# ru-wang/slam-plus-plus

Measured on AMD Instinct MI355X. Metric: Λ-solve block-nnz/sec + batch GN iters/sec, Venice BA, 1→8 MI355X, higher is better.
Workload: dtype f64; 1 GPU; venice871-shaped synthetic BA (871 cams, 530304 points, 2838740 observations, LM-damped); nnzb=3369915, n=1596138, mode=schur+dense, n_reduced=5226, schur_pairs=12875640, parallelism=single GPU

## Files before the change

### include/spp_hip.h

```cpp
#ifndef SPP_HIP_H
#define SPP_HIP_H

#include <stddef.h>
#include <stdint.h>

#ifdef __cplusplus
extern "C" {
#endif

#define SPP_OK            0
#define SPP_NOT_POSDEF    1
#define SPP_E_BADARG     -1
#define SPP_E_NOMEM      -2
#define SPP_E_HIP        -3
#define SPP_E_NO_DEVICE  -4
#define SPP_E_STATE      -5
#define SPP_E_UNSUPPORTED -6

#define SPP_MODE_AUTO     0
#define SPP_MODE_SPARSE   1
#define SPP_MODE_SCHUR    2
#define SPP_MODE_SCHUR_SPARSE 3

#define SPP_FLAG_PROFILE  1
// ... 3 lines not shown

spp_ctx *spp_create(int device, int flags);
void spp_destroy(spp_ctx *ctx);
int spp_free_memory(spp_ctx *ctx);
int spp_last_error(const spp_ctx *ctx, char *buf, size_t buf_size);
double *spp_host_staging(spp_ctx *ctx, int64_t n_doubles);
int spp_set_stream(spp_ctx *ctx, void *hip_stream);
int spp_synchronize(spp_ctx *ctx);

int spp_analyze(spp_ctx *ctx, int64_t nb, const int64_t *h_col_ptr, const int64_t *h_row_idx,
	const int64_t *h_blk_off, const int32_t *h_dim, int mode);

int spp_set_shard(spp_ctx *ctx, int rank, int world_size);

#define SPP_MODE_SCHUR_MIS 4

#define SPP_INFO_MODE           0
#define SPP_INFO_N              1
#define SPP_INFO_NNZB           2
#define SPP_INFO_NVALS          3
#define SPP_INFO_FACTOR_NNZ     4
#define SPP_INFO_FACTOR_FLOPS   5
#define SPP_INFO_N_REDUCED      6
#define SPP_INFO_N_POSES        7
#define SPP_INFO_N_LANDMARKS    8
#define SPP_INFO_SCHUR_PAIRS    9
#define SPP_INFO_N_OBS          10
#define SPP_INFO_SOLVE_BYTES    11
#define SPP_INFO_N_SUPERNODES   12
#define SPP_INFO_N_LEVELS       13
#define SPP_INFO_S_LD           14
#define SPP_INFO_S_NNZB         15
#define SPP_INFO_DENSE_STREAMED 16
int spp_get_info(const spp_ctx *ctx, int what, int64_t *out);
int spp_get_ordering(const spp_ctx *ctx, int64_t *h_order);

#define SPP_ORDER_AMD 0
#define SPP_ORDER_ND  1
int spp_block_ordering(int64_t nb, const int64_t *col_ptr, const int64_t *row_idx, int method, int64_t *h_order);

int spp_schur_plan_host(int64_t nb, const int32_t *dim, const int64_t *col_ptr, const int64_t *row_idx, int shard_rank,
	int shard_world, int sparse_S, int64_t *out, double *seconds);

int spp_factor_solve(spp_ctx *ctx, const double *h_vals, double *h_rhs_inout);

int spp_factor_solve_device(spp_ctx *ctx, const double *d_vals, double *d_rhs_inout);

int spp_schur_buffer_size(const spp_ctx *ctx, int64_t *n_doubles);
int spp_schur_form(spp_ctx *ctx, const double *d_vals, const double *d_rhs, double *d_S_rhs);
int spp_schur_finish(spp_ctx *ctx, const double *d_vals, double *d_S_rhs, double *d_rhs_inout);
int spp_schur_packed_size(const spp_ctx *ctx, int64_t *n_doubles);
int spp_schur_pack(spp_ctx *ctx, const double *d_S_rhs, double *d_packed);
int spp_schur_unpack(spp_ctx *ctx, const double *d_packed, double *d_S_rhs);

int spp_assemble_analyze(spp_ctx *ctx, int64_t nv, const int32_t *h_dim,
	int64_t ne, const int64_t *h_v0, const int64_t *h_v1, int d0, int d1, int rd,
	int64_t unary_vertex);
int spp_assemble_get_structure(const spp_ctx *ctx, int64_t *h_col_ptr, int64_t *h_row_idx,
	int64_t *h_blk_off);
int spp_assemble_device(spp_ctx *ctx, const double *d_J0, const double *d_J1,
	const double *d_Omega, const double *d_r, double damping, double *d_vals_out, double *d_eta_out);
int spp_assemble_set_edge_weights(spp_ctx *ctx, const double *d_w);
int spp_edge_robust_weights_device(spp_ctx *ctx, int64_t n_edges, int rd, int kind, double scale, double param,
	const double *d_r, double *d_w_out);

int spp_se2_linearize_device(spp_ctx *ctx, int64_t n_edges, const int32_t *d_v0, const int32_t *d_v1,
// ... 72 lines not shown
```

### slam_plus_plus_amd/api.py

```python
import ctypes
import os

import numpy as np

_HERE = os.path.dirname(os.path.abspath(__file__))
LIB_PATH = os.environ.get("SPP_LIB") or os.path.join(_HERE, "libspp_hip.so")

SPP_OK, SPP_NOT_POSDEF = 0, 1
MODE_AUTO, MODE_SPARSE, MODE_SCHUR, MODE_SCHUR_SPARSE, MODE_SCHUR_MIS = 0, 1, 2, 3, 4
FLAG_PROFILE = 1
INFO = dict(MODE=0, N=1, NNZB=2, NVALS=3, FACTOR_NNZ=4, FACTOR_FLOPS=5, N_REDUCED=6, N_POSES=7,
            N_LANDMARKS=8, SCHUR_PAIRS=9, N_OBS=10, SOLVE_BYTES=11, N_SUPERNODES=12, N_LEVELS=13, S_LD=14, S_NNZB=15, DENSE_STREAMED=16)
PHASES = ["permute", "schur_inv", "schur_gemm", "schur_rhs", "factor", "trisolve", "backsubst", "assemble", "total"]

EXPORTS = [
    "spp_create", "spp_destroy", "spp_free_memory", "spp_last_error", "spp_host_staging", "spp_set_stream", "spp_synchronize",
    "spp_analyze", "spp_set_shard", "spp_get_info", "spp_get_ordering", "spp_factor_solve",
    "spp_factor_solve_device", "spp_schur_buffer_size", "spp_schur_form", "spp_schur_finish",
    "spp_schur_packed_size", "spp_schur_pack", "spp_schur_unpack",
    "spp_assemble_analyze", "spp_assemble_get_structure", "spp_assemble_device", "spp_assemble_set_edge_weights", "spp_device_malloc",
    "spp_device_free", "spp_memcpy_h2d", "spp_memcpy_d2h", "spp_memcpy_d2d", "spp_get_phase_ms", "spp_get_dominant_kernel",
    "spp_microbench_copy", "spp_microbench_mfma_f64", "spp_microbench_ctile", "spp_microbench_update", "spp_block_ordering", "spp_schur_plan_host", "spp_set_profiling", "spp_se2_linearize_device", "spp_se2_update_device", "spp_ba_linearize_device", "spp_ba_update_device", "spp_se3_linearize_device", "spp_se3_update_device", "spp_edge_chi2_device", "spp_edge_robust_weights_device", "spp_edge_hessian_maxdiag_device",
    "spp_lm_gain_denominator_device", "spp_dense_potrf_upper", "spp_dense_posv",
    "spp_dense_posv_masked", "spp_tile_mask_host", "spp_schur_tile_mask_host", "spp_tail_order_host", "spp_schur_cam_order_host",
    "spp_dense_gemm_tn_sub", "spp_dense_gemm_tn_sub_upper", "spp_dense_front_factor", "spp_version",
]

_lib = None
_c_i64p = ctypes.POINTER(ctypes.c_int64)
_c_i32p = ctypes.POINTER(ctypes.c_int32)
_c_f64p = ctypes.POINTER(ctypes.c_double)


class SppError(RuntimeError):
    """std::runtime_error of the C++ adapter (reference LinearSolver_Schur_GPU.cpp:734-797)."""


def load_library():
    global _lib
    if _lib is not None:
        return _lib
    if not os.path.exists(LIB_PATH):
        raise SppError("libspp_hip.so is not built: run `python -m slam_plus_plus_amd.build` "
                       "(hipcc --offload-arch=gfx950); there is no CPU fallback")
    lib = ctypes.CDLL(LIB_PATH)
# ... 444 lines not shown
```

### slam_plus_plus_amd/csrc/spp_api.cpp

```cpp

#include "spp_internal.h"
#include <string.h>
#include <new>

using namespace spp;

namespace spp {

void phases_reset(spp_ctx *ctx)
{
	if(!(ctx->flags & SPP_FLAG_PROFILE))
		return;
	if(!ctx->timer.created) {
		for(int i = 0; i < 2 * SPP_N_PHASES; ++ i)
			SPP_HIP_CHECK(hipEventCreate(&ctx->timer.ev[i]));
		ctx->timer.created = true;
	}
	for(int i = 0; i < SPP_N_PHASES; ++ i) {
		ctx->timer.used[i] = false;
		ctx->phase_ms[i] = 0;
	}
	ctx->dom_used = 0;
	ctx->dom_flops = 0;
}
// ... 326 lines not shown
	} else
		sparse_analyze(ctx, ctx->st);
	ctx->mode = chosen;
	clk.lap("plan + ordering");
	return SPP_OK;
	SPP_CATCH(ctx)
}

int spp_get_info(const spp_ctx *ctx, int what, int64_t *out)
{
	if(!ctx || !out)
		return SPP_E_BADARG;
	if(ctx->mode < 0 && what != SPP_INFO_NNZB && what != SPP_INFO_NVALS && what != SPP_INFO_N && what != SPP_INFO_DENSE_STREAMED)
		return SPP_E_STATE;
	switch(what) {
	case SPP_INFO_MODE: *out = (ctx->mode != SPP_MODE_SCHUR) ? ctx->mode : ctx->schur.mis ? SPP_MODE_SCHUR_MIS :
		ctx->schur.sparse_S ? SPP_MODE_SCHUR_SPARSE : SPP_MODE_SCHUR; break;
	case SPP_INFO_N: *out = ctx->st.n; break;
	case SPP_INFO_NNZB: *out = ctx->st.nnzb; break;
	case SPP_INFO_NVALS: *out = ctx->st.nvals; break;
	case SPP_INFO_FACTOR_NNZ: *out = ctx->factor_nnz; break;
	case SPP_INFO_FACTOR_FLOPS: *out = ctx->factor_flops; break;
	case SPP_INFO_N_REDUCED: *out = (ctx->mode == SPP_MODE_SCHUR) ? ctx->schur.n_red : 0; break;
	case SPP_INFO_N_POSES: *out = (ctx->mode == SPP_MODE_SCHUR) ? ctx->schur.nc : ctx->st.nb; break;
	case SPP_INFO_N_LANDMARKS: *out = (ctx->mode == SPP_MODE_SCHUR) ? ctx->schur.nl : 0; break;
	case SPP_INFO_SCHUR_PAIRS: *out = (ctx->mode == SPP_MODE_SCHUR) ? ctx->schur.n_pairs : 0; break;
	case SPP_INFO_N_OBS: *out = (ctx->mode == SPP_MODE_SCHUR) ? ctx->schur.no : 0; break;
	case SPP_INFO_SOLVE_BYTES: *out = ctx->solve_bytes; break;
	case SPP_INFO_N_SUPERNODES: *out = ctx->sparse ? sparse_info(ctx, what) : 0; break;
	case SPP_INFO_N_LEVELS: *out = ctx->sparse ? sparse_info(ctx, what) : 0; break;
	case SPP_INFO_S_LD: *out = (ctx->mode == SPP_MODE_SCHUR && !ctx->schur.sparse_S) ? ctx->schur.ld : 0; break;
	case SPP_INFO_S_NNZB: *out = (ctx->mode == SPP_MODE_SCHUR) ? ctx->schur.n_sblk : 0; break;
	case SPP_INFO_DENSE_STREAMED: *out = ctx->dense.tail_rows_last; break;
	default: return SPP_E_BADARG;
	}
	return SPP_OK;
}

int spp_get_ordering(const spp_ctx *ctx, int64_t *h_order)
{
	if(!ctx || !h_order)
		return SPP_E_BADARG;
	if(ctx->mode < 0)
		return SPP_E_STATE;
	for(size_t i = 0; i < ctx->order.size(); ++ i)
		h_order[i] = ctx->order[i];
	return SPP_OK;
}

int spp_block_ordering(int64_t nb, const int64_t *col_ptr, const int64_t *row_idx, int method, int64_t *h_order)
{
	if(nb <= 0 || !col_ptr || !row_idx || !h_order || (method != SPP_ORDER_AMD && method != SPP_ORDER_ND))
		return SPP_E_BADARG;
	try {
		for(int64_t j = 0; j < nb; ++ j)
			for(int64_t p = col_ptr[j]; p < col_ptr[j + 1]; ++ p)
				if(row_idx[p] < 0 || row_idx[p] > j)
					return SPP_E_BADARG;
		std::vector<int64_t> order;
		if(method == SPP_ORDER_AMD)
			min_degree_order(nb, col_ptr, row_idx, order);
		else
			nested_dissection_order(nb, col_ptr, row_idx, order);
		for(int64_t k = 0; k < nb; ++ k)
			h_order[k] = order[k];
		return SPP_OK;
// ... 692 lines not shown
```

### slam_plus_plus_amd/csrc/spp_internal.h

```cpp
#pragma once

#include <hip/hip_runtime.h>
#include <stdint.h>
#include <string>
#include <vector>
#include <sys/mman.h>
#include <utility>
#include <new>
#include <exception>
#include <thread>
#include <stdexcept>
#include <algorithm>
#include <string.h>
#include <chrono>
#include <stdio.h>
#include <stdlib.h>
#include "../../include/spp_hip.h"
#include "spp_switches.h"

namespace spp {

struct Error : std::runtime_error {
	int code;
	Error(int c, const std::string &what) : std::runtime_error(what), code(c) {}
// ... 152 lines not shown
	int32_t kind;
	int32_t a_tr;
	int64_t dst;
	int64_t aoff;
};

struct SchurDims {
	int dp = 0, dl = 0;
	int64_t nc = 0, nl = 0;
	int64_t nl_total = 0;
	int64_t no = 0;
	int64_t n_red = 0, ld = 0;
	int64_t n_sblk = 0;
	int64_t n_pairs = 0;
	int64_t n_items = 0, n_multi = 0;
	int32_t xcd_max_items = 0;
	bool u_landmark_major = true;
	bool factored = true;
};

struct SchurPlan : SchurDims {
	bool add_A = true;
	bool sparse_S = false;
	bool mis = false;
	Structure s_st;
	DevBuf<int64_t> sblk_voff;
	std::vector<int64_t> pose_block;
	std::vector<int64_t> lm_block;
	std::vector<uint8_t> is_lm;
	std::vector<uint64_t> tile_mask;
	DevBuf<int32_t> lm_ptr;
	DevBuf<int32_t> bs_ptr;
	int64_t n_bs = 0;
	DevBuf<int64_t> lm_coff;
	DevBuf<int64_t> lm_rbase;
	DevBuf<int32_t> obs_pose;
	DevBuf<int32_t> obs_lm;
	DevBuf<int64_t> obs_off;
	DevBuf<int64_t> pose_rbase;
	DevBuf<int32_t> cam_ptr;
	DevBuf<int32_t> cam_obs;
	DevBuf<int32_t> obs_wpos;
	DevBuf<SaccItem> items;
	DevBuf<int32_t> xcd_beg;
	DevBuf<int32_t> sblk_i1, sblk_i2;
	DevBuf<int64_t> sblk_aoff;
	DevBuf<int32_t> pair_a, pair_b;
	DevBuf<int32_t> multi_blk;
	DevBuf<int32_t> multi_ptr;
	DevBuf<double> cinv;
	DevBuf<double> lfac;
	DevBuf<double> W;
	DevBuf<double> Up;
	DevBuf<double> xw;
	DevBuf<double> partial;
	DevBuf<double> S;
	void release_all();
};

struct DenseWork {
	DevBuf<double> tinv;
	DevBuf<int> info;
	DevBuf<double> tinv_all;
	int64_t tinv_half = 0;
	DevBuf<double> xtmp;
	DevBuf<int> flags;
// ... 210 lines not shown
```

### slam_plus_plus_amd/csrc/spp_schur.hip

```cpp

#include "spp_internal.h"

namespace spp {

template <int DL>
__device__ __forceinline__ void cinv_block(const double *__restrict__ m, double *o)
{
	if(DL == 3) {
#define M_(i, j) m[(i) + 3 * (j)]
#define COF_(i, j) (M_(((i) + 1) % 3, ((j) + 1) % 3) * M_(((i) + 2) % 3, ((j) + 2) % 3) - \
	M_(((i) + 1) % 3, ((j) + 2) % 3) * M_(((i) + 2) % 3, ((j) + 1) % 3))
		const double c00 = COF_(0, 0), c10 = COF_(1, 0), c20 = COF_(2, 0);
		const double det = c00 * M_(0, 0) + c10 * M_(1, 0) + c20 * M_(2, 0);
		const double id = -1.0 / det;
		o[0] = c00 * id; o[3] = c10 * id; o[6] = c20 * id;
		o[1] = COF_(0, 1) * id; o[4] = COF_(1, 1) * id; o[7] = COF_(2, 1) * id;
		o[2] = COF_(0, 2) * id; o[5] = COF_(1, 2) * id; o[8] = COF_(2, 2) * id;
#undef COF_
#undef M_
	} else if(DL == 2) {
		const double det = m[0] * m[3] - m[2] * m[1];
		const double id = -1.0 / det;
		o[0] = m[3] * id; o[2] = -m[2] * id;
		o[1] = -m[1] * id; o[3] = m[0] * id;
// ... 250 lines not shown
#pragma unroll
	for(int q = 0; q < DL; ++ q)
#pragma unroll
		for(int r = 0; r < DP; ++ r) {
			double sum = 0;
#pragma unroll
			for(int t = 0; t < DL; ++ t)
				if(t <= q)
					sum += U[r + DP * t] * F[t + DL * q];
			V[r + DP * q] = sum;
			Wl[r] -= sum * tv[q];
		}
#pragma unroll
	for(int e = 0; e < BLK; ++ e)
		img[lane * ST + e] = V[e];
	__syncthreads();
	for(int p = lane; p < nact * IL; p += 64) {
		const int j = p / IL, e = p - j * IL;
		Vm[a0 * IL + p] = img[j * ST + e];
	}
	if(SIDE)
		for(int p = lane; p < nact * SIDE; p += 64) {
			const int j = p / (SIDE ? SIDE : 1), e = p - j * SIDE;
			Vs[a0 * SIDE + p] = img[j * ST + IL + e];
		}
	__syncthreads();
#pragma unroll
	for(int r = 0; r < DP; ++ r)
		img[lane * (DP | 1) + r] = Wl[r];
	__syncthreads();
	for(int p = lane; p < nact * DP; p += 64) {
		const int j = p / DP, r = p - j * DP;
		xw[(int64_t)slot[j] * DP + r] = img[j * (DP | 1) + r];
	}
}

constexpr int SACC_WAVES = 4;
#ifndef SPP_SACC_RP
#define SPP_SACC_RP 64
#endif
#ifndef SPP_SACC_UCOL
#define SPP_SACC_UCOL 0
#endif
#ifndef SPP_SACC_GLDS
#define SPP_SACC_GLDS 1
#endif

__device__ __forceinline__ SaccItem sacc_load_item(const SaccItem *__restrict__ items, int32_t idx, int32_t lim)
{
	SaccItem r;
	r.beg = r.end = 0;
	r.kind = -1;
	r.a_tr = 0;
	r.dst = 0;
	r.aoff = -1;
	if(idx < lim)
		r = items[idx];
	return r;
}

#ifndef SPP_SACC_EU
#define SPP_SACC_EU 2
#endif
template <int DP, int DL, bool FACT>
__global__ __launch_bounds__(SACC_WAVES * 64) __attribute__((amdgpu_waves_per_eu(SPP_SACC_EU, SPP_SACC_EU)))
void s_accum_kernel(const SaccItem *__restrict__ items, const int32_t *__restrict__ xcd_beg, int chunk,
// ... 249 lines not shown
		pa = pa_n;
		pb = pb_n;
	}
}

template <int DP>
__global__ __launch_bounds__(256)
void s_multi_kernel(int64_t n_multi, const int32_t *__restrict__ multi_blk, const int32_t *__restrict__ multi_ptr,
	const int32_t *__restrict__ sblk_i1, const int32_t *__restrict__ sblk_i2, const int64_t *__restrict__ sblk_aoff,
	const double *__restrict__ partial, const double *__restrict__ vals, int add_A, double *__restrict__ S, int64_t ld,
	const int64_t *__restrict__ sblk_voff)
{
	const int64_t m = (int64_t)blockIdx.x * (blockDim.x >> 6) + (threadIdx.x >> 6);
	const int lane = threadIdx.x & 63;
	if(m >= n_multi || lane >= DP * DP)
		return;
	const int32_t b = multi_blk[m];
	double acc = 0;
	for(int32_t s = multi_ptr[m]; s < multi_ptr[m + 1]; ++ s)
		acc += partial[(int64_t)s * DP * DP + lane];
	const int64_t aoff = sblk_aoff[b];
	if(add_A && aoff >= 0)
		acc = vals[aoff + lane] + acc;
	else if(add_A && aoff < -1)
		acc = vals[(-2 - aoff) + lane / DP + (lane % DP) * DP] + acc;
	if(sblk_voff) {
		S[sblk_voff[b] + lane] = acc;
		return;
	}
	const int r = lane % DP, c = lane / DP;
	S[((int64_t)sblk_i1[b] * DP + r) + ((int64_t)sblk_i2[b] * DP + c) * ld] = acc;
}

template <int DP>
__global__ __launch_bounds__(256)
void rhs_kernel(int64_t nc, const int32_t *__restrict__ cam_ptr, const int32_t *__restrict__ cam_obs,
	const int64_t *__restrict__ pose_rbase, const double *__restrict__ xw, const double *__restrict__ rhs,
	int add_eta, double *__restrict__ xcol)
{
	const int64_t i = (int64_t)blockIdx.x * (blockDim.x >> 6) + (threadIdx.x >> 6);
	const int lane = threadIdx.x & 63;
	if(i >= nc)
		return;
	double s[DP];
#pragma unroll
	for(int r = 0; r < DP; ++ r)
		s[r] = 0;
	for(int32_t q = cam_ptr[i] + lane; q < cam_ptr[i + 1]; q += 64) {
		const double *x = xw + (int64_t)q * DP;
#pragma unroll
		for(int r = 0; r < DP; ++ r)
			s[r] += x[r];
	}
#pragma unroll
	for(int r = 0; r < DP; ++ r) {
#pragma unroll
		for(int off = 32; off > 0; off >>= 1)
			s[r] += __shfl_xor(s[r], off);
	}
	if(lane < DP) {
		double v = 0;
#pragma unroll
		for(int r = 0; r < DP; ++ r)
			if(lane == r)
				v = s[r];
		if(add_eta)
			v += rhs[pose_rbase[i] + lane];
		xcol[i * DP + lane] = v;
	}
}

template <int DP, int DL>
__global__ __launch_bounds__(256)
void backsubst_obs_kernel(int64_t no, const int32_t *__restrict__ obs_pose, const int64_t *__restrict__ obs_off,
	const double *__restrict__ vals, const double *__restrict__ dx, double *__restrict__ tq)
{
	const int64_t a = (int64_t)blockIdx.x * blockDim.x + threadIdx.x;
	if(a >= no)
		return;
	double u[DP * DL];
	load_U<DP, DL>(vals, obs_off[a], u);
	double dv[DP];
// ... 76 lines not shown
		}
	}
	__syncthreads();
	if(t >= l1 - l0)
		return;
	const int64_t l = (int64_t)l0 + t;
	double tv[DL];
	const int64_t rb = lm_rbase[l];
#pragma unroll
	for(int q = 0; q < DL; ++ q)
		tv[q] = -rhs[rb + q];
	for(int32_t a = lm_ptr[l] - a0, e = lm_ptr[l + 1] - a0; a < e; ++ a) {
#pragma unroll
		for(int q = 0; q < DL; ++ q)
			tv[q] += tq[a * DL + q];
	}
	double Ci[DL * DL];
	if(cinv) {
#pragma unroll
		for(int e = 0; e < DL * DL; ++ e)
			Ci[e] = cinv[l * DL * DL + e];
	} else
		cinv_block<DL>(vals + lm_coff[l], Ci);
#pragma unroll
	for(int q = 0; q < DL; ++ q) {
		double sum = 0;
#pragma unroll
		for(int u = 0; u < DL; ++ u)
			sum += Ci[q + DL * u] * tv[u];
		rhs[rb + q] = sum;
	}
}

template <int DP>
__global__ __launch_bounds__(256)
void scatter_dx_kernel(int64_t nc, const int64_t *__restrict__ pose_rbase, const double *__restrict__ dx,
	double *__restrict__ rhs)
{
	const int64_t e = (int64_t)blockIdx.x * blockDim.x + threadIdx.x;
	if(e >= nc * DP)
		return;
	rhs[pose_rbase[e / DP] + e % DP] = dx[e];
}

template <int DP, int DL>
static void schur_form_t(spp_ctx *ctx, const double *d_vals, const double *d_rhs, double *S)
{
	SchurPlan &sp = ctx->schur;
	hipStream_t s = ctx->stream;
	const int64_t ld = sp.ld;
	const int64_t *voff = sp.sparse_S ? sp.sblk_voff.p : nullptr;
	double *xcol = sp.sparse_S ? S + sp.s_st.nvals : S + sp.n_red * ld;
	phase_begin(ctx, SPP_PHASE_SCHUR_INV);
	if(S == sp.S.p && !sp.sparse_S && ctx->shard_world == 1 && sp.n_sblk == sp.nc * (sp.nc + 1) / 2 && sp.n_red == sp.nc * DP)
		SPP_HIP_CHECK(hipMemsetAsync(S + sp.n_red * ld, 0, (size_t)(schur_buffer_doubles(ctx) - sp.n_red * ld) * sizeof(double), s));
	else
		SPP_HIP_CHECK(hipMemsetAsync(S, 0, (size_t)schur_buffer_doubles(ctx) * sizeof(double), s));
	constexpr int VIL = VSplit<DP * DL>::IL;
	double *Vm = sp.W.p, *Vs = sp.W.p + sp.no * VIL;
	const bool onfly = sp.factored && DL <= 3;
	if(sp.nl && !onfly)
		hipLaunchKernelGGL((cinv_kernel<DL>), dim3((unsigned)((sp.nl + 255) / 256)), dim3(256), 0, s,
			sp.nl, sp.lm_coff.p, d_vals, sp.cinv.p, sp.factored ? sp.lfac.p : nullptr);
	if(sp.no && sp.factored)
		hipLaunchKernelGGL((obs_fact_kernel<DP, DL>), dim3((unsigned)((sp.no + 255) / 256)), dim3(256), 0, s,
			sp.no, sp.obs_lm.p, sp.obs_off.p, sp.lm_rbase.p, d_vals, d_rhs, onfly ? (const double*)nullptr : (const double*)sp.lfac.p, sp.lm_coff.p,
			sp.obs_wpos.p, Vm, Vs, sp.xw.p);
	else if(sp.no)
		hipLaunchKernelGGL((obs_kernel<DP, DL>), dim3((unsigned)((sp.no + 255) / 256)), dim3(256), 0, s,
			sp.no, sp.obs_lm.p, sp.obs_off.p, sp.lm_rbase.p, d_vals, d_rhs, sp.cinv.p, sp.obs_wpos.p, sp.W.p, sp.Up.p, sp.xw.p, sp.u_landmark_major ? 1 : 0);
	phase_end(ctx, SPP_PHASE_SCHUR_INV);
	phase_begin(ctx, SPP_PHASE_SCHUR_GEMM);
	if(sp.n_items) {
		int chunk = switches().sacc_chunk;
		if(chunk <= 0)
			chunk = (int)((sp.xcd_max_items + SACC_WAVES * 64 - 1) / (SACC_WAVES * 64));
		const int64_t per = (int64_t)SACC_WAVES * chunk;
		if(sp.factored)
			hipLaunchKernelGGL((s_accum_kernel<DP, DL, true>), dim3((unsigned)(8 * ((sp.xcd_max_items + per - 1) / per))), dim3(SACC_WAVES * 64), 0, s,
				sp.items.p, sp.xcd_beg.p, chunk, sp.pair_a.p, sp.pair_b.p, Vm, Vs, d_vals, S, ld, sp.partial.p);
		else
			hipLaunchKernelGGL((s_accum_kernel<DP, DL, false>), dim3((unsigned)(8 * ((sp.xcd_max_items + per - 1) / per))), dim3(SACC_WAVES * 64), 0, s,
				sp.items.p, sp.xcd_beg.p, chunk, sp.pair_a.p, sp.pair_b.p, sp.W.p, sp.Up.p, d_vals, S, ld, sp.partial.p);
	}
	if(sp.n_multi)
		hipLaunchKernelGGL((s_multi_kernel<DP>), dim3((unsigned)((sp.n_multi + 3) / 4)), dim3(256), 0, s,
			sp.n_multi, sp.multi_blk.p, sp.multi_ptr.p, sp.sblk_i1.p, sp.sblk_i2.p, sp.sblk_aoff.p,
			sp.partial.p, d_vals, sp.add_A ? 1 : 0, S, ld, voff);
	phase_end(ctx, SPP_PHASE_SCHUR_GEMM);
	phase_begin(ctx, SPP_PHASE_SCHUR_RHS);
	if(sp.nc)
		hipLaunchKernelGGL((rhs_kernel<DP>), dim3((unsigned)((sp.nc + 3) / 4)), dim3(256), 0, s,
			sp.nc, sp.cam_ptr.p, sp.cam_obs.p, sp.pose_rbase.p, sp.xw.p, d_rhs, sp.add_A ? 1 : 0, xcol);
	phase_end(ctx, SPP_PHASE_SCHUR_RHS);
	SPP_HIP_CHECK(hipGetLastError());
}

template <int DP, int DL>
static int schur_finish_t(spp_ctx *ctx, const double *d_vals, double *S, double *d_rhs)
{
	SchurPlan &sp = ctx->schur;
	hipStream_t s = ctx->stream;
	const int64_t ld = sp.ld;
	double *xcol;
	if(sp.sparse_S) {
		xcol = S + sp.s_st.nvals;
		const int ret = sparse_factor_solve(ctx, S, xcol);
		if(ret != SPP_OK)
			return ret;
	} else {
		phase_begin(ctx, SPP_PHASE_FACTOR);
		dense_set_padding(ctx, S, ld, sp.n_red);
		{
			TileMaskGuard guard(ctx->dense, &sp.tile_mask);
			dense_potrf_upper_enqueue(ctx, S, sp.n_red, ld);
		}
		phase_end(ctx, SPP_PHASE_FACTOR);
		xcol = S + sp.n_red * ld;
		phase_begin(ctx, SPP_PHASE_TRISOLVE);
		dense_potrs_upper(ctx, S, sp.n_red, ld, xcol);
		phase_end(ctx, SPP_PHASE_TRISOLVE);
	}
	phase_begin(ctx, SPP_PHASE_BACKSUBST);
	static_assert(DL <= DP, "the products U^T dx reuse the W l buffer (DP doubles per observation)");
	const int bs_fused = switches().backsubst_fused;
	const double *cinv_arg = (sp.factored && DL <= 3) ? (const double*)nullptr : (const double*)sp.cinv.p;
	if(bs_fused && sp.n_bs > 0)
		hipLaunchKernelGGL((backsubst_fused_kernel<DP, DL>), dim3((unsigned)sp.n_bs), dim3(256), 0, s,
			sp.bs_ptr.p, sp.lm_ptr.p, sp.obs_pose.p, sp.obs_off.p, sp.lm_rbase.p, cinv_arg, sp.lm_coff.p, d_vals, xcol, d_rhs);
	else {
		if(sp.no)
			hipLaunchKernelGGL((backsubst_obs_kernel<DP, DL>), dim3((unsigned)((sp.no + 255) / 256)), dim3(256), 0, s,
				sp.no, sp.obs_pose.p, sp.obs_off.p, d_vals, xcol, sp.xw.p);
		if(sp.nl)
			hipLaunchKernelGGL((backsubst_lm_kernel<DL>), dim3((unsigned)((sp.nl + 255) / 256)), dim3(256), 0, s,
				sp.nl, sp.lm_ptr.p, sp.lm_rbase.p, sp.xw.p, cinv_arg, sp.lm_coff.p, d_vals, d_rhs);
	}
	if(sp.nc)
		hipLaunchKernelGGL((scatter_dx_kernel<DP>), dim3((unsigned)((sp.nc * DP + 255) / 256)), dim3(256), 0, s,
			sp.nc, sp.pose_rbase.p, xcol, d_rhs);
	phase_end(ctx, SPP_PHASE_BACKSUBST);
	SPP_HIP_CHECK(hipGetLastError());
	if(!sp.sparse_S && dense_info_fetch(ctx))
		return SPP_NOT_POSDEF;
	return SPP_OK;
}

template <bool PACK>
__global__ __launch_bounds__(256)
void schur_pack_kernel(double *__restrict__ S, int64_t ld, double *__restrict__ packed)
{
	const int64_t k = blockIdx.y;
	const int64_t rows = 128 * (k + 1);
	const int64_t e = (int64_t)blockIdx.x * 256 + threadIdx.x;
	if(e >= rows * 128)
		return;
	const int64_t r = e % rows, c = e / rows;
	double *ps = S + r + (128 * k + c) * ld;
	double *pp = packed + 128 * 128 * (k * (k + 1) / 2) + e;
	if(PACK)
// ... 38 lines not shown
```

### slam_plus_plus_amd/csrc/spp_switches.h

```cpp
#pragma once

#include <stdint.h>
#include <stdlib.h>
#include <string.h>
#include <algorithm>

namespace spp {

constexpr long long WAIT_TICKS_PER_MS = 100000;
constexpr long long WAIT_TICKS_DEFAULT = 500 * WAIT_TICKS_PER_MS;

enum Ordering { ORDERING_AUTO, ORDERING_AMD, ORDERING_ND };
constexpr int MID_FRONT_MAX = 640;

struct Switches {
	bool verbose;
	int plan_threads;
	int64_t plan_min_work;

	int dense_sched;
	int fused;
	int aux_reserve_cus;
	int tile_444;
	int dense_la;
	int la_chain_mask;
	int la_g2;
	int la_bulk_acquire;
	int64_t la_slots;
	int la_trace;
	int tail_rows;
	int tail_mask;
	double tail_order_beta;
	int tail_early;
	long long tail_timeout_ticks;
	int tail_trace;
	int trsv_chain;
	int trsv_mform;

	bool sacc_ulm;
	bool sacc_factored;
	int64_t sacc_tile;
	int64_t sacc_tile_cols;
	int sacc_xcd;
	int sacc_chunk;
	int schur_cam_order;
	int backsubst_fused;

	int mid_front_max;
	Ordering ordering;
	int64_t amalg_small;
	double amalg_zeros;
	int64_t amalg_relax_h;
	double amalg_zeros_small;
	bool sparse_teams;
	int sparse_team_max;
	int sparse_team_cols;
	int sparse_dag;
	int dag_split;
	long long dag_timeout_ticks;
	int dag_trace;
};

inline int env_int(const char *name, int dflt)
{
	const char *e = getenv(name);
	return e ? atoi(e) : dflt;
}

inline long long env_i64(const char *name, long long dflt)
{
	const char *e = getenv(name);
	return e ? atoll(e) : dflt;
}

inline double env_double(const char *name, double dflt)
{
	const char *e = getenv(name);
	return e ? atof(e) : dflt;
}
// ... 3 lines not shown
	Switches w;
	w.verbose = getenv("SPP_VERBOSE") != nullptr;
	const char *threads = getenv("SPP_PLAN_THREADS");
	w.plan_threads = threads ? std::max(1, atoi(threads)) : 0;
	w.plan_min_work = std::max<int64_t>(1, env_i64("SPP_PLAN_MIN_WORK", int64_t(1) << 18));

	w.dense_sched = env_int("SPP_DENSE_SCHED", 1);
	w.fused = env_int("SPP_FUSED", 1);
	w.aux_reserve_cus = env_int("SPP_AUX_RESERVE_CUS", 32);
	w.tile_444 = env_int("SPP_TILE_444", 0);
	w.dense_la = env_int("SPP_DENSE_LA", 0);
	w.la_chain_mask = env_int("SPP_LA_CHAIN_MASK", 1);
	w.la_g2 = env_int("SPP_LA_G2", 0);
	w.la_bulk_acquire = env_int("SPP_LA_BULK_ACQUIRE", 1);
	w.la_slots = env_i64("SPP_LA_SLOTS", 0);
	w.la_trace = env_int("SPP_LA_TRACE", 0);
	w.tail_rows = env_int("SPP_DENSE_TAIL", 1) ? env_int("SPP_TAIL_ROWS", 44) : 0;
	w.tail_mask = env_int("SPP_TAIL_MASK", 1);
	w.tail_order_beta = env_double("SPP_TAIL_ORDER_BETA", 0.0);
	w.tail_early = env_int("SPP_TAIL_EARLY", 1);
	w.tail_timeout_ticks = env_i64("SPP_TAIL_TIMEOUT_TICKS", WAIT_TICKS_DEFAULT);
	w.tail_trace = env_int("SPP_TAIL_TRACE", 0);
	w.trsv_chain = env_int("SPP_TRSV_CHAIN", 2);
	w.trsv_mform = env_int("SPP_TRSV_MFORM", 1);

	w.sacc_ulm = env_int("SPP_SACC_ULM", 1) != 0;
	w.sacc_factored = env_int("SPP_SACC_FACTORED", 1) != 0;
	w.sacc_tile = std::max<int64_t>(1, env_i64("SPP_SACC_TILE", 4));
	w.sacc_tile_cols = env_i64("SPP_SACC_TILE_COLS", -2);
	w.sacc_xcd = env_int("SPP_SACC_XCD", 1);
	w.sacc_chunk = env_int("SPP_SACC_CHUNK", 1);
	w.schur_cam_order = env_int("SPP_SCHUR_CAM_ORDER", 1);
	w.backsubst_fused = env_int("SPP_BACKSUBST_FUSED", 1);

	w.mid_front_max = std::max(128, std::min(MID_FRONT_MAX, env_int("SPP_MID_FRONT_MAX", 320)));
	const char *ordering = getenv("SPP_ORDERING");
	w.ordering = !ordering ? ORDERING_AUTO : (!strcmp(ordering, "nd") ? ORDERING_ND : ORDERING_AMD);
	w.amalg_small = env_i64("SPP_AMALG_SMALL", 32);
	w.amalg_zeros = env_double("SPP_AMALG_ZEROS", 0.12);
	w.amalg_relax_h = env_i64("SPP_AMALG_RELAX_H", 96);
	w.amalg_zeros_small = env_double("SPP_AMALG_ZEROS_SMALL", 0.2);
	w.sparse_teams = env_int("SPP_SPARSE_TEAMS", 1) != 0;
	w.sparse_team_max = std::max(1, std::min(64, env_int("SPP_SPARSE_TEAM_MAX", 40)));
	w.sparse_team_cols = std::max(8, std::min(256, env_int("SPP_SPARSE_TEAM_COLS", 16)));
	w.sparse_dag = env_int("SPP_SPARSE_DAG", 1);
	w.dag_split = env_int("SPP_DAG_SPLIT", 1);
	w.dag_timeout_ticks = env_i64("SPP_DAG_TIMEOUT_TICKS", WAIT_TICKS_DEFAULT);
	w.dag_trace = env_int("SPP_DAG_TRACE", 0);
	return w;
}

inline const Switches &switches()
{
	static const Switches w = parse_switches();
	return w;
}

}
```

Before: 1.266 billion block-nnz/s.

## Add coalesced LDS-staged streaming kernels for Schur observation factor and back-substitution

Adds a wave-cooperative obs_fact_stream kernel that loads the 6x3 observation blocks as coalesced 16-byte pieces through LDS, transposes them in registers, and writes Vm/Vs/xw back with vectorised stores. The xw buffer can be indexed by observation instead of by camera position, and rhs_kernel gathers through cam_obs when that layout is used. A new backsubst_stream kernel processes several landmark groups per block and prefetches the next group's blocks while the current one is reduced. The intent is to replace strided per-thread global loads with coalesced traffic and to hide load latency. The cost is more LDS, more barriers, and an indirect gather in the RHS reduction.

```diff
diff --git a/include/spp_hip.h b/include/spp_hip.h
--- a/include/spp_hip.h
+++ b/include/spp_hip.h
@@ -59,6 +59,8 @@
 #define SPP_INFO_S_LD           14
 #define SPP_INFO_S_NNZB         15
 #define SPP_INFO_DENSE_STREAMED 16
+#define SPP_INFO_LM_STREAM      17
+#define SPP_INFO_BS_GROUPS      18
 int spp_get_info(const spp_ctx *ctx, int what, int64_t *out);
 int spp_get_ordering(const spp_ctx *ctx, int64_t *h_order);
 
diff --git a/slam_plus_plus_amd/api.py b/slam_plus_plus_amd/api.py
--- a/slam_plus_plus_amd/api.py
+++ b/slam_plus_plus_amd/api.py
@@ -10,7 +10,8 @@
 MODE_AUTO, MODE_SPARSE, MODE_SCHUR, MODE_SCHUR_SPARSE, MODE_SCHUR_MIS = 0, 1, 2, 3, 4
 FLAG_PROFILE = 1
 INFO = dict(MODE=0, N=1, NNZB=2, NVALS=3, FACTOR_NNZ=4, FACTOR_FLOPS=5, N_REDUCED=6, N_POSES=7,
-            N_LANDMARKS=8, SCHUR_PAIRS=9, N_OBS=10, SOLVE_BYTES=11, N_SUPERNODES=12, N_LEVELS=13, S_LD=14, S_NNZB=15, DENSE_STREAMED=16)
+            N_LANDMARKS=8, SCHUR_PAIRS=9, N_OBS=10, SOLVE_BYTES=11, N_SUPERNODES=12, N_LEVELS=13, S_LD=14, S_NNZB=15, DENSE_STREAMED=16,
+            LM_STREAM=17, BS_GROUPS=18)
 PHASES = ["permute", "schur_inv", "schur_gemm", "schur_rhs", "factor", "trisolve", "backsubst", "assemble", "total"]
 
 EXPORTS = [
diff --git a/slam_plus_plus_amd/csrc/spp_api.cpp b/slam_plus_plus_amd/csrc/spp_api.cpp
--- a/slam_plus_plus_amd/csrc/spp_api.cpp
+++ b/slam_plus_plus_amd/csrc/spp_api.cpp
@@ -382,6 +382,8 @@
 	case SPP_INFO_S_LD: *out = (ctx->mode == SPP_MODE_SCHUR && !ctx->schur.sparse_S) ? ctx->schur.ld : 0; break;
 	case SPP_INFO_S_NNZB: *out = (ctx->mode == SPP_MODE_SCHUR) ? ctx->schur.n_sblk : 0; break;
 	case SPP_INFO_DENSE_STREAMED: *out = ctx->dense.tail_rows_last; break;
+	case SPP_INFO_LM_STREAM: *out = (ctx->mode == SPP_MODE_SCHUR) ? ctx->schur.lm_stream_last : 0; break;
+	case SPP_INFO_BS_GROUPS: *out = (ctx->mode == SPP_MODE_SCHUR) ? ctx->schur.n_bs : 0; break;
 	default: return SPP_E_BADARG;
 	}
 	return SPP_OK;
diff --git a/slam_plus_plus_amd/csrc/spp_internal.h b/slam_plus_plus_amd/csrc/spp_internal.h
--- a/slam_plus_plus_amd/csrc/spp_internal.h
+++ b/slam_plus_plus_amd/csrc/spp_internal.h
@@ -208,6 +208,7 @@
 	DevBuf<int32_t> lm_ptr;
 	DevBuf<int32_t> bs_ptr;
 	int64_t n_bs = 0;
+	int lm_stream_last = 0;
 	DevBuf<int64_t> lm_coff;
 	DevBuf<int64_t> lm_rbase;
 	DevBuf<int32_t> obs_pose;
diff --git a/slam_plus_plus_amd/csrc/spp_schur.hip b/slam_plus_plus_amd/csrc/spp_schur.hip
--- a/slam_plus_plus_amd/csrc/spp_schur.hip
+++ b/slam_plus_plus_amd/csrc/spp_schur.hip
@@ -306,6 +306,147 @@
 	for(int p = lane; p < nact * DP; p += 64) {
 		const int j = p / DP, r = p - j * DP;
 		xw[(int64_t)slot[j] * DP + r] = img[j * (DP | 1) + r];
+	}
+}
+
+typedef double dbl2_a8 __attribute__((ext_vector_type(2), aligned(8)));
+typedef double dbl2_a16 __attribute__((ext_vector_type(2), aligned(16)));
+
+__device__ __forceinline__ void wave_lds_sync()
+{
+	__builtin_amdgcn_fence(__ATOMIC_ACQ_REL, "wavefront");
+	__builtin_amdgcn_wave_barrier();
+}
+
+template <int BLK>
+__device__ __forceinline__ void fetch_U_pieces(const double *__restrict__ vals, const int64_t *off, int nact, int lane, dbl2_a8 *pc)
+{
+	constexpr int NP = BLK / 2;
+#pragma unroll
+	for(int k = 0; k < NP; ++ k) {
+		const int p = lane + 64 * k, j = p / NP, e = p - j * NP;
+		pc[k] = *(const dbl2_a8*)(vals + (off[(j < nact) ? j : nact - 1] >> 1) + 2 * e);
+	}
+}
+
+template <int BLK>
+__device__ __forceinline__ void store_U_pieces(double *img, int lane, const dbl2_a8 *pc)
+{
+	constexpr int NP = BLK / 2, ST = BLK | 1;
+#pragma unroll
+	for(int k = 0; k < NP; ++ k) {
+		const int p = lane + 64 * k, j = p / NP, e = p - j * NP;
+		img[j * ST + 2 * e] = pc[k].x;
+		img[j * ST + 2 * e + 1] = pc[k].y;
+	}
+}
+
+template <int DP, int DL>
+__device__ __forceinline__ void take_U(const double *row, bool transposed, double *U)
+{
+	if(transposed) {
+#pragma unroll
+		for(int r = 0; r < DP; ++ r)
+#pragma unroll
+			for(int q = 0; q < DL; ++ q)
+				U[r + DP * q] = row[q + DL * r];
+	} else {
+#pragma unroll
+		for(int e = 0; e < DP * DL; ++ e)
+			U[e] = row[e];
+	}
+}
+
+template <int DP, int DL, bool XW_OBS>
+__global__ __launch_bounds__(256)
+void obs_fact_stream_kernel(int64_t no, const int32_t *__restrict__ obs_lm, const int64_t *__restrict__ obs_off,
+	const int64_t *__restrict__ lm_rbase, const double *__restrict__ vals, const double *__restrict__ rhs,
+	const double *__restrict__ lfac, const int64_t *__restrict__ lm_coff, const int32_t *__restrict__ obs_wpos, double *__restrict__ Vm, double *__restrict__ Vs,
+	double *__restrict__ xw)
+{
+	constexpr int BLK = DP * DL, ST = BLK | 1, IL = VSplit<BLK>::IL, SIDE = VSplit<BLK>::SIDE, XST = DP | 1;
+	static_assert(BLK % 2 == 0 && IL % 2 == 0 && SIDE % 2 == 0 && DP % 2 == 0, "16-byte pieces");
+	__shared__ double img_all[4][64 * ST];
+	__shared__ int64_t off_all[4][64];
+	const int lane = threadIdx.x & 63, wave = threadIdx.x >> 6;
+	double *img = img_all[wave];
+	int64_t *off = off_all[wave];
+	const int64_t a0 = ((int64_t)blockIdx.x * 4 + wave) * 64, a = a0 + lane;
+	if(a0 >= no)
+		return;
+	const bool active = a < no;
+	const int nact = (no - a0 < 64) ? (int)(no - a0) : 64;
+	const int64_t oo = active ? obs_off[a] : 0;
+	const int32_t l = active ? obs_lm[a] : 0;
+	const int64_t rb = lm_rbase[l], coff = lm_coff[l];
+	off[lane] = oo;
+	wave_lds_sync();
+	dbl2_a8 pc[BLK / 2];
+	fetch_U_pieces<BLK>(vals, off, nact, lane, pc);
+	double F[DL * DL], lv[DL], tv[DL];
+	if(lfac) {
+#pragma unroll
+		for(int e = 0; e < DL * DL; ++ e)
+			F[e] = lfac[(int64_t)l * DL * DL + e];
+	} else
+		lfac_block<DL>(vals + coff, F);
+#pragma unroll
+	for(int q = 0; q < DL; ++ q)
+		lv[q] = rhs[rb + q];
+#pragma unroll
+	for(int q = 0; q < DL; ++ q) {
+		double sum = 0;
+#pragma unroll
+		for(int u = 0; u < DL; ++ u)
+			if(u <= q)
+				sum += F[u + DL * q] * lv[u];
+		tv[q] = sum;
+	}
+	store_U_pieces<BLK>(img, lane, pc);
+	wave_lds_sync();
+	double U[BLK];
+	take_U<DP, DL>(img + lane * ST, (oo & 1) != 0, U);
+	double V[BLK], Wl[DP];
+#pragma unroll
+	for(int r = 0; r < DP; ++ r)
+		Wl[r] = 0;
+#pragma unroll
+	for(int q = 0; q < DL; ++ q)
+#pragma unroll
+		for(int r = 0; r < DP; ++ r) {
+			double sum = 0;
+#pragma unroll
+			for(int t = 0; t < DL; ++ t)
+				if(t <= q)
+					sum += U[r + DP * t] * F[t + DL * q];
+			V[r + DP * q] = sum;
+			Wl[r] -= sum * tv[q];
+		}
+#pragma unroll
+	for(int e = 0; e < BLK; ++ e)
+		img[lane * ST + e] = V[e];
+	wave_lds_sync();
+	for(int p = lane; p < nact * (IL / 2); p += 64) {
+		const int j = p / (IL / 2), e = p - j * (IL / 2);
+		const dbl2_a16 v = {img[j * ST + 2 * e], img[j * ST + 2 * e + 1]};
+		*(dbl2_a16*)(Vm + a0 * IL + 2 * p) = v;
+	}
+	if(SIDE)
+		for(int p = lane; p < nact * (SIDE / 2); p += 64) {
+			const int j = p / (SIDE ? SIDE / 2 : 1), e = p - j * (SIDE / 2);
+			const dbl2_a16 v = {img[j * ST + IL + 2 * e], img[j * ST + IL + 2 * e + 1]};
+			*(dbl2_a16*)(Vs + a0 * SIDE + 2 * p) = v;
+		}
+	wave_lds_sync();
+#pragma unroll
+	for(int r = 0; r < DP; ++ r)
+		img[lane * XST + r] = Wl[r];
+	wave_lds_sync();
+	for(int p = lane; p < nact * (DP / 2); p += 64) {
+		const int j = p / (DP / 2), e = p - j * (DP / 2);
+		const dbl2_a16 v = {img[j * XST + 2 * e], img[j * XST + 2 * e + 1]};
+		const int64_t row = XW_OBS ? a0 + j : (int64_t)obs_wpos[a0 + j];
+		*(dbl2_a16*)(xw + row * DP + 2 * e) = v;
 	}
 }
 
@@ -621,7 +762,7 @@
 	S[((int64_t)sblk_i1[b] * DP + r) + ((int64_t)sblk_i2[b] * DP + c) * ld] = acc;
 }
 
-template <int DP>
+template <int DP, bool XW_OBS>
 __global__ __launch_bounds__(256)
 void rhs_kernel(int64_t nc, const int32_t *__restrict__ cam_ptr, const int32_t *__restrict__ cam_obs,
 	const int64_t *__restrict__ pose_rbase, const double *__restrict__ xw, const double *__restrict__ rhs,
@@ -635,8 +776,9 @@
 #pragma unroll
 	for(int r = 0; r < DP; ++ r)
 		s[r] = 0;
+#pragma unroll 4
 	for(int32_t q = cam_ptr[i] + lane; q < cam_ptr[i + 1]; q += 64) {
-		const double *x = xw + (int64_t)q * DP;
+		const double *x = xw + (int64_t)(XW_OBS ? cam_obs[q] : q) * DP;
 #pragma unroll
 		for(int r = 0; r < DP; ++ r)
 			s[r] += x[r];
@@ -779,6 +921,110 @@
 	}
 }
 
+template <int DP, int DL>
+__global__ __launch_bounds__(256)
+void backsubst_stream_kernel(int32_t n_bs, int32_t per, const int32_t *__restrict__ bs_ptr, const int32_t *__restrict__ lm_ptr, const int32_t *__restrict__ obs_pose,
+	const int64_t *__restrict__ obs_off, const int64_t *__restrict__ lm_rbase, const double *__restrict__ cinv,
+	const int64_t *__restrict__ lm_coff, const double *__restrict__ vals, const double *__restrict__ dx, double *__restrict__ rhs)
+{
+	constexpr int BLK = DP * DL, ST = BLK | 1;
+	static_assert(BLK % 2 == 0, "16-byte pieces");
+	__shared__ double img_all[4][64 * ST];
+	__shared__ int64_t off_all[4][64];
+	__shared__ double tq_all[2][256 * DL];
+	const int t = threadIdx.x, lane = t & 63, wave = t >> 6;
+	double *img = img_all[wave];
+	int64_t *off = off_all[wave];
+	const int32_t g0 = blockIdx.x * per, g1 = (g0 + per < n_bs) ? g0 + per : n_bs;
+	dbl2_a8 pc[BLK / 2] = {};
+	double dv[DP];
+	int32_t l0, l1, a0, na;
+	bool transposed;
+	auto request = [&](int32_t g) {
+		l0 = bs_ptr[g], l1 = bs_ptr[g + 1];
+		a0 = lm_ptr[l0], na = lm_ptr[l1] - a0;
+		const int64_t oo = (t < na) ? obs_off[(int64_t)a0 + t] : 0;
+		const double *d = dx + (int64_t)((t < na) ? obs_pose[(int64_t)a0 + t] : 0) * DP;
+		transposed = (oo & 1) != 0;
+		off[lane] = oo;
+		wave_lds_sync();
+#pragma unroll
+		for(int r = 0; r < DP; ++ r)
+			dv[r] = d[r];
+		const int rest = na - 64 * wave;
+		if(rest > 0)
+			fetch_U_pieces<BLK>(vals, off, (rest < 64) ? rest : 64, lane, pc);
+	};
+	if(g0 < g1)
+		request(g0);
+	for(int32_t g = g0; g < g1; ++ g) {
+		double *tq = tq_all[(g - g0) & 1];
+		store_U_pieces<BLK>(img, lane, pc);
+		wave_lds_sync();
+		if(t < na) {
+			double u[BLK];
+			take_U<DP, DL>(img + lane * ST, transposed, u);
+#pragma unroll
+			for(int q = 0; q < DL; ++ q) {
+				double sum = 0;
+#pragma unroll
+				for(int r = 0; r < DP; ++ r)
+					sum += dv[r] * u[r + DP * q];
+				tq[t * DL + q] = sum;
+			}
+		}
+		const int32_t nlg = l1 - l0, ga0 = a0;
+		const bool lm_lane = t < nlg;
+		const int64_t l = (int64_t)l0 + (lm_lane ? t : 0);
+		const int64_t rb = lm_rbase[l];
+		const int32_t pa = lm_ptr[l] - ga0, pe = lm_ptr[l + 1] - ga0;
+		double tv[DL], m[DL * DL];
+#pragma unroll
+		for(int q = 0; q < DL; ++ q)
+			tv[q] = -rhs[rb + q];
+		{
+			const double *src = cinv ? cinv + l * DL * DL : vals + lm_coff[l];
+#pragma unroll
+			for(int e = 0; e < DL * DL; ++ e)
+				m[e] = src[e];
+		}
+		if(g + 1 < g1)
+			request(g + 1);
+		else {
+#pragma unroll
+			for(int q = 0; q < DL; ++ q)
+				asm volatile("" : "+v"(tv[q]));
+#pragma unroll
+			for(int e = 0; e < DL * DL; ++ e)
+				asm volatile("" : "+v"(m[e]));
+			asm volatile("" :: "v"(pa), "v"(pe));
+		}
+		asm volatile("s_waitcnt lgkmcnt(0)\n\ts_barrier" ::: "memory");
+		if(lm_lane) {
+			for(int32_t p = pa; p < pe; ++ p) {
+#pragma unroll
+				for(int q = 0; q < DL; ++ q)
+					tv[q] += tq[p * DL + q];
+			}
+			double Ci[DL * DL];
+			if(cinv) {
+#pragma unroll
+				for(int e = 0; e < DL * DL; ++ e)
+					Ci[e] = m[e];
+			} else
+				cinv_block<DL>(m, Ci);
+#pragma unroll
+			for(int q = 0; q < DL; ++ q) {
+				double sum = 0;
+#pragma unroll
+				for(int u = 0; u < DL; ++ u)
+					sum += Ci[q + DL * u] * tv[u];
+				rhs[rb + q] = sum;
+			}
+		}
+	}
+}
+
 template <int DP>
 __global__ __launch_bounds__(256)
 void scatter_dx_kernel(int64_t nc, const int64_t *__restrict__ pose_rbase, const double *__restrict__ dx,
@@ -788,6 +1034,33 @@
 	if(e >= nc * DP)
 		return;
 	rhs[pose_rbase[e / DP] + e % DP] = dx[e];
+}
+
+template <int DP, int DL>
+static int lm_stream_form(const SchurPlan &sp)
+{
+	if(!(DP == 6 && DL == 3) || !sp.factored)
+		return 0;
+	const int v = switches().lm_stream;
+	return (v == 1 || v == 2) ? v : 0;
+}
+
+template <int DP, int DL, typename... Args>
+static void launch_obs_fact_stream(bool xw_obs, dim3 grid, hipStream_t s, Args... args)
+{
+	if constexpr(DP == 6 && DL == 3) {
+		if(xw_obs)
+			hipLaunchKernelGGL((obs_fact_stream_kernel<DP, DL, true>), grid, dim3(256), 0, s, args...);
+		else
+			hipLaunchKernelGGL((obs_fact_stream_kernel<DP, DL, false>), grid, dim3(256), 0, s, args...);
+	}
+}
+
+template <int DP, int DL, typename... Args>
+static void launch_backsubst_stream(dim3 grid, hipStream_t s, Args... args)
+{
+	if constexpr(DP == 6 && DL == 3)
+		hipLaunchKernelGGL((backsubst_stream_kernel<DP, DL>), grid, dim3(256), 0, s, args...);
 }
 
 template <int DP, int DL>
@@ -809,12 +1082,19 @@
 	if(sp.nl && !onfly)
 		hipLaunchKernelGGL((cinv_kernel<DL>), dim3((unsigned)((sp.nl + 255) / 256)), dim3(256), 0, s,
 			sp.nl, sp.lm_coff.p, d_vals, sp.cinv.p, sp.factored ? sp.lfac.p : nullptr);
-	if(sp.no && sp.factored)
-		hipLaunchKernelGGL((obs_fact_kernel<DP, DL>), dim3((unsigned)((sp.no + 255) / 256)), dim3(256), 0, s,
-			sp.no, sp.obs_lm.p, sp.obs_off.p, sp.lm_rbase.p, d_vals, d_rhs, onfly ? (const double*)nullptr : (const double*)sp.lfac.p, sp.lm_coff.p,
+	const int lm_stream = lm_stream_form<DP, DL>(sp);
+	sp.lm_stream_last = lm_stream;
+	const double *lfac_arg = onfly ? (const double*)nullptr : (const double*)sp.lfac.p;
+	const dim3 obs_grid((unsigned)((sp.no + 255) / 256));
+	if(sp.no && lm_stream)
+		launch_obs_fact_stream<DP, DL>(lm_stream == 1, obs_grid, s, sp.no, sp.obs_lm.p, sp.obs_off.p, sp.lm_rbase.p, d_vals, d_rhs, lfac_arg,
+			sp.lm_coff.p, sp.obs_wpos.p, Vm, Vs, sp.xw.p);
+	else if(sp.no && sp.factored)
+		hipLaunchKernelGGL((obs_fact_kernel<DP, DL>), obs_grid, dim3(256), 0, s,
+			sp.no, sp.obs_lm.p, sp.obs_off.p, sp.lm_rbase.p, d_vals, d_rhs, lfac_arg, sp.lm_coff.p,
 			sp.obs_wpos.p, Vm, Vs, sp.xw.p);
 	else if(sp.no)
-		hipLaunchKernelGGL((obs_kernel<DP, DL>), dim3((unsigned)((sp.no + 255) / 256)), dim3(256), 0, s,
+		hipLaunchKernelGGL((obs_kernel<DP, DL>), obs_grid, dim3(256), 0, s,
 			sp.no, sp.obs_lm.p, sp.obs_off.p, sp.lm_rbase.p, d_vals, d_rhs, sp.cinv.p, sp.obs_wpos.p, sp.W.p, sp.Up.p, sp.xw.p, sp.u_landmark_major ? 1 : 0);
 	phase_end(ctx, SPP_PHASE_SCHUR_INV);
 	phase_begin(ctx, SPP_PHASE_SCHUR_GEMM);
@@ -836,8 +1116,11 @@
 			sp.partial.p, d_vals, sp.add_A ? 1 : 0, S, ld, voff);
 	phase_end(ctx, SPP_PHASE_SCHUR_GEMM);
 	phase_begin(ctx, SPP_PHASE_SCHUR_RHS);
-	if(sp.nc)
-		hipLaunchKernelGGL((rhs_kernel<DP>), dim3((unsigned)((sp.nc + 3) / 4)), dim3(256), 0, s,
+	if(sp.nc && lm_stream == 1)
+		hipLaunchKernelGGL((rhs_kernel<DP, true>), dim3((unsigned)((sp.nc + 3) / 4)), dim3(256), 0, s,
+			sp.nc, sp.cam_ptr.p, sp.cam_obs.p, sp.pose_rbase.p, sp.xw.p, d_rhs, sp.add_A ? 1 : 0, xcol);
+	else if(sp.nc)
+		hipLaunchKernelGGL((rhs_kernel<DP, false>), dim3((unsigned)((sp.nc + 3) / 4)), dim3(256), 0, s,
 			sp.nc, sp.cam_ptr.p, sp.cam_obs.p, sp.pose_rbase.p, sp.xw.p, d_rhs, sp.add_A ? 1 : 0, xcol);
 	phase_end(ctx, SPP_PHASE_SCHUR_RHS);
 	SPP_HIP_CHECK(hipGetLastError());
@@ -872,7 +1155,12 @@
 	static_assert(DL <= DP, "the products U^T dx reuse the W l buffer (DP doubles per observation)");
 	const int bs_fused = switches().backsubst_fused;
 	const double *cinv_arg = (sp.factored && DL <= 3) ? (const double*)nullptr : (const double*)sp.cinv.p;
-	if(bs_fused && sp.n_bs > 0)
+	const int32_t bs_per = (sp.n_bs >= 1024) ? 4 : 1;
+	if(bs_fused && sp.n_bs > 0 && lm_stream_form<DP, DL>(sp))
+		launch_backsubst_stream<DP, DL>(dim3((unsigned)((sp.n_bs + bs_per - 1) / bs_per)), s,
+			(int32_t)sp.n_bs, bs_per, (const int32_t*)sp.bs_ptr.p, (const int32_t*)sp.lm_ptr.p, (const int32_t*)sp.obs_pose.p, (const int64_t*)sp.obs_off.p,
+			(const int64_t*)sp.lm_rbase.p, cinv_arg, (const int64_t*)sp.lm_coff.p, d_vals, (const double*)xcol, d_rhs);
+	else if(bs_fused && sp.n_bs > 0)
 		hipLaunchKernelGGL((backsubst_fused_kernel<DP, DL>), dim3((unsigned)sp.n_bs), dim3(256), 0, s,
 			sp.bs_ptr.p, sp.lm_ptr.p, sp.obs_pose.p, sp.obs_off.p, sp.lm_rbase.p, cinv_arg, sp.lm_coff.p, d_vals, xcol, d_rhs);
 	else {
diff --git a/slam_plus_plus_amd/csrc/spp_switches.h b/slam_plus_plus_amd/csrc/spp_switches.h
--- a/slam_plus_plus_amd/csrc/spp_switches.h
+++ b/slam_plus_plus_amd/csrc/spp_switches.h
@@ -45,6 +45,7 @@
 	int sacc_chunk;
 	int schur_cam_order;
 	int backsubst_fused;
+	int lm_stream;
 
 	int mid_front_max;
 	Ordering ordering;
@@ -114,6 +115,7 @@
 	w.sacc_chunk = env_int("SPP_SACC_CHUNK", 1);
 	w.schur_cam_order = env_int("SPP_SCHUR_CAM_ORDER", 1);
 	w.backsubst_fused = env_int("SPP_BACKSUBST_FUSED", 1);
+	w.lm_stream = env_int("SPP_LM_STREAM", 1);
 
 	w.mid_front_max = std::max(128, std::min(MID_FRONT_MAX, env_int("SPP_MID_FRONT_MAX", 320)));
 	const char *ordering = getenv("SPP_ORDERING");
```

After: 1.296 billion block-nnz/s (median of 6 runs). +2.3%, better.
